# pdlfs/old-vpic

Measured on AMD Instinct MI355X. Metric: particle-pushes/sec (full step: advance_p + sort when due + field solve + glue), higher is better.
Workload: dtype f32

## Files before the change

### old-vpic_amd/csrc/push.hip

```cpp
#include "push_device.h"
#include "record_offsets.h"
#include <cstdlib>
#include <cstring>
#include <cstddef>
#include <vector>
#include <algorithm>

namespace vpichip {

struct PushParams {
  float qdt_2mc, cdt_dx, cdt_dy, cdt_dz;
  int np;
  int iters;
  int sy, sz;
  int idx_base;
  unsigned *crossed;
  const int *tpart, *ttail; int ntx, nty, ntiles, n_sorted; unsigned mul_sy, sh_sy, mul_sz, sh_sz;
  const int *tile_list; int n_launch, tail_chunks;
  int nx, ny, nz;
  int follow;
  double acc_scale;
  int *hist; int ntz;
  ParticlesK out; int *next;
  int stage;
// ... 63 lines not shown
struct MissList { int key[MISS_CAP]; float v[MISS_CAP][12]; int total; };

__device__ __forceinline__ void flush_misses(MissList *ml, int &n_miss, float *g_acc, int lane) {
  if (n_miss > 0) {
    __builtin_amdgcn_fence(__ATOMIC_ACQ_REL, "workgroup");
    const int entry = lane / 12, k = lane - entry * 12;
    if (entry < n_miss) atomicAdd(g_acc + (size_t)ml->key[entry] * 12 + k, ml->v[entry][k]);
    if (lane == 0) ml->total += n_miss;
    __builtin_amdgcn_fence(__ATOMIC_ACQ_REL, "workgroup");
    n_miss = 0;
  }
}

struct HistK { int *hist; unsigned *s_cnt; TileK tk; };
template <class W>
__device__ __forceinline__ void hist_count(const HistK &h, int key, int wbase, int sy, int sz, const TileDiv &td) {
  const int slot = slot_of<W>(key, wbase, sy, sz, td);
  if (slot >= 0) atomicAdd(&h.s_cnt[slot >> 1], 1u << ((slot & 1) << 4));
  else atomicAdd(&h.hist[sort_key<true>(key, h.tk)], 1);
}

template <class W>
__device__ __forceinline__ void deposit_run(const bool tail, float (&a)[12], int key, int lane, typename W::acc_t *s_acc, float *g_acc,
                                            int wbase, int sy, int sz, const TileDiv &td, MissList *ml, int &n_miss, const int pre_slot = -2) {
  const int slot = pre_slot != -2 ? pre_slot : slot_of<W>(key, wbase, sy, sz, td);
  if constexpr (is_det<W>::value) {
    if (tail) deposit12<true, W>(s_acc, g_acc, key, slot, a, td.scale);
    return;
  }
  if (tail && slot >= 0) deposit12<true, W>(s_acc, g_acc, key, slot, a);
  const bool miss = tail && slot < 0;
  const unsigned long long mm = __ballot(miss);
  if (mm) {
    if (miss) moments_to_terms(a, a);
    const int cnt = __popcll(mm);
    if (cnt > MISS_CAP) {
      if (miss) deposit12<true, W>(s_acc, g_acc, key, -1, a);
      if (lane == 0) ml->total += cnt;
      } else {
      if (n_miss + cnt > MISS_CAP) flush_misses(ml, n_miss, g_acc, lane);
      if (miss) {
        const int e = n_miss + mbcnt64(mm);
        ml->key[e] = key;
#pragma unroll
        for (int k = 0; k < 12; k++) ml->v[e][k] = a[k];
      }
      n_miss += cnt;
    }
  }
}

template <int BLOCK, class W>
__device__ __forceinline__ void run_deposit(float (&a)[12], int key, int lane, typename W::acc_t *s_acc, float *g_acc,
                                            int wbase, int sy, int sz, const TileDiv &td, MissList *ml, int &n_miss,
                                            const HistK *hk = nullptr, const bool counted = false, const int given_slot = -2) {
  static_assert(BLOCK == 1 || BLOCK == 2 || BLOCK == 4 || BLOCK == 8 || BLOCK == 16 || BLOCK == 64, "scan width");
  if (BLOCK == 1) {
    deposit_run<W>(key >= 0, a, key, lane, s_acc, g_acc, wbase, sy, sz, td, ml, n_miss);
    return;
  }
  const int prev = __builtin_amdgcn_update_dpp(-2, key, 0x138 , 0xf, 0xf, false);
  const unsigned long long block_heads = BLOCK == 64 ? 0ull : BLOCK == 16 ? 0x0001000100010001ull : BLOCK == 8 ? 0x0101010101010101ull
                                       : BLOCK == 4 ? 0x1111111111111111ull : 0x5555555555555555ull;
  const unsigned long long heads = __ballot(prev != key) | block_heads;
  const unsigned long long below = heads & ((2ull << lane) - 1ull);
  const int d = lane - (63 - __clzll((long long)below));
  const float f1 = d >= 1 ? 1.f : 0.f;
  SEG_STEP12(a, f1, "row_shr:1 row_mask:0xf bank_mask:0xf bound_ctrl:1");
  if (BLOCK >= 4) {
    const float f2 = d >= 2 ? 1.f : 0.f;
    SEG_STEP12(a, f2, "row_shr:2 row_mask:0xf bank_mask:0xf bound_ctrl:1");
  }
  if (BLOCK >= 8) {
    const float f4 = d >= 4 ? 1.f : 0.f;
    SEG_STEP12(a, f4, "row_shr:4 row_mask:0xf bank_mask:0xf bound_ctrl:1");
  }
  if (BLOCK >= 16) {
    const float f8 = d >= 8 ? 1.f : 0.f;
    SEG_STEP12(a, f8, "row_shr:8 row_mask:0xf bank_mask:0xf bound_ctrl:1");
  }
  if (BLOCK == 64) {
    const int r = lane & 15;
    const float f16 = d > r ? 1.f : 0.f;
    const float f32 = d > (lane & 31) ? 1.f : 0.f;
    SEG_STEP12(a, f16, "row_bcast:15 row_mask:0xa bank_mask:0xf");
    SEG_STEP12(a, f32, "row_bcast:31 row_mask:0xc bank_mask:0xf");
  }
  asm volatile("s_nop 1");
  const bool tail = (lane == 63) || ((heads >> ((lane + 1) & 63)) & 1ull);
  if (hk) {
    const int slot = slot_of<W>(key, wbase, sy, sz, td);
    const unsigned long long inc = __ballot(counted);
    const unsigned long long run = ((2ull << lane) - 1ull) & ~((1ull << (lane - d)) - 1ull);
    const int n = __popcll(inc & run);
    if (tail && key >= 0 && n) {
      if (slot >= 0) atomicAdd(&hk->s_cnt[slot >> 1], (unsigned)n << ((slot & 1) << 4));
      else atomicAdd(&hk->hist[sort_key<true>(key, hk->tk)], n);
    }
    deposit_run<W>(tail && key >= 0, a, key, lane, s_acc, g_acc, wbase, sy, sz, td, ml, n_miss, slot);
    return;
  }
  deposit_run<W>(tail && key >= 0, a, key, lane, s_acc, g_acc, wbase, sy, sz, td, ml, n_miss, given_slot);
}

template <int BLOCK, class W>
__device__ __forceinline__ void run_deposit_fixed(const float (&a)[12], int key, int lane, typename W::acc_t *s_acc, float *g_acc,
                                                  int wbase, int sy, int sz, const TileDiv &td, MissList *ml, int &n_miss) {
  static_assert(BLOCK == 16, "runs of at most 16 lanes, within a DPP row");
  unsigned long long v[12];
#pragma unroll
  for (int k = 0; k < 12; k++) v[k] = to_fixed(a[k], td.scale);
  const int prev = __builtin_amdgcn_update_dpp(-2, key, 0x138 , 0xf, 0xf, false);
  const unsigned long long heads = __ballot(prev != key) | 0x0001000100010001ull;
  const unsigned long long below = heads & ((2ull << lane) - 1ull);
  const int d = lane - (63 - __clzll((long long)below));
#pragma unroll
  for (int step = 1; step < 16; step <<= 1) {
    const bool on = d >= step;
#pragma unroll
    for (int k = 0; k < 12; k++) {
      const int lo = (int)(unsigned)v[k], hi = (int)(unsigned)(v[k] >> 32);
      const int tl = step == 1 ? __builtin_amdgcn_update_dpp(0, lo, 0x111 , 0xf, 0xf, true)
                   : step == 2 ? __builtin_amdgcn_update_dpp(0, lo, 0x112, 0xf, 0xf, true)
                   : step == 4 ? __builtin_amdgcn_update_dpp(0, lo, 0x114, 0xf, 0xf, true)
                               : __builtin_amdgcn_update_dpp(0, lo, 0x118, 0xf, 0xf, true);
      const int th = step == 1 ? __builtin_amdgcn_update_dpp(0, hi, 0x111, 0xf, 0xf, true)
                   : step == 2 ? __builtin_amdgcn_update_dpp(0, hi, 0x112, 0xf, 0xf, true)
                   : step == 4 ? __builtin_amdgcn_update_dpp(0, hi, 0x114, 0xf, 0xf, true)
                               : __builtin_amdgcn_update_dpp(0, hi, 0x118, 0xf, 0xf, true);
      const unsigned long long t = ((unsigned long long)(unsigned)th << 32) | (unsigned long long)(unsigned)tl;
      v[k] += on ? t : 0ull;
    }
  }
  const bool tail = key >= 0 && ((lane == 63) || ((heads >> ((lane + 1) & 63)) & 1ull));
  if (tail) {
    const int slot = slot_of<W>(key, wbase, sy, sz, td);
    unsigned long long *g64 = reinterpret_cast<unsigned long long *>(g_acc) + (size_t)key * 12;
#pragma unroll
    for (int k = 0; k < 12; k++) {
      if (slot >= 0) atomicAdd(&s_acc[k * W::NSLOT_PAD + slot], v[k]); else atomicAdd(&g64[k], v[k]);
    }
  }
  asm volatile("" ::: "memory");
}

constexpr int WAVES = PUSH_THREADS / 64;

#ifndef VPIC_HIP_MQW
#define VPIC_HIP_MQW 64
#endif
static_assert(VPIC_HIP_MQW >= 64, "a pass can yield 64 cell-crossers: the queue must hold them once it has been drained");
constexpr int MQW = VPIC_HIP_MQW;
struct WaveQueue { float4 pos_i[MQW]; float4 disp_idx[MQW]; float q[MQW]; };
constexpr int FLIP_SHIFT = 28;

__device__ __forceinline__ float fast_rsq(float x) { return __builtin_amdgcn_rsqf(x); }
__device__ __forceinline__ float fast_rcp(float x) { return __builtin_amdgcn_rcpf(x); }

template <class W>
__device__ __forceinline__ void mover_streak12(float *a, float q, float mx, float my, float mz, float sx, float sy, float sz) {
  if constexpr (is_det<W>::value) {
    const float v5 = (float)((double)(q * sx * sy * sz) * (1. / 3.));
    streak12(a, q, mx, my, mz, sx, sy, sz, v5);
  } else {
    streak12_moments(a, q, mx, my, mz, sx, sy, sz);
  }
}

constexpr int STAGE_CAP = 2;
template <bool CHARGELESS> struct StageRounds { static constexpr int value = CHARGELESS ? 2 : 1; };
struct StagePark { int base[STAGE_CAP], qb[STAGE_CAP]; unsigned cm_lo[STAGE_CAP], cm_hi[STAGE_CAP], act_lo[STAGE_CAP], act_hi[STAGE_CAP]; };
constexpr int STAGED_BIT = 31;
struct Straggler { float4 pos_i, disp_idx; float q; bool live; unsigned long long again; };

template <bool FAST, class W, bool HIST = false, bool STAGE = false, bool WIDE = false>
__device__ __forceinline__ int drain_wave(const ParticlesK &p, const int rel, WaveQueue *mq, const int n_mq,
                                          const int lane, typename W::acc_t *s_acc, float *g_acc, const int wbase,
                                          const DrainParams *dp, const int ablate, const int max_round, const int idx_base,
                                          MissList *ml, int &n_miss, const double det_scale = 0, const HistK *hk = nullptr, Straggler *sg = nullptr) {
  if (ablate & 64) return 0;
  typedef int int8v __attribute__((ext_vector_type(8)));
  typedef int int4v __attribute__((ext_vector_type(4)));
  int8v d0, d1; int4v d2;
  asm volatile("s_load_dwordx8 %0, %3, 0x0\n\ts_load_dwordx8 %1, %3, 0x20\n\ts_load_dwordx4 %2, %3, 0x40\n\ts_waitcnt lgkmcnt(0)"
               : "=&s"(d0), "=&s"(d1), "=&s"(d2) : "s"(dp));
  static_assert(offsetof(DrainParams, pbc) == 0x20 && offsetof(DrainParams, pm) == 0x40 && sizeof(DrainParams) == 0x50, "DrainParams layout");
  const int gnx = d0[0], gny = d0[1], gnz = d0[2], gsy = d0[3], gsz = d0[4], grank = d0[5], max_nm = d0[6];
  const unsigned mul_sz = (unsigned)d0[7], mul_sy = (unsigned)d1[6], sh_sz = (unsigned)d1[7] >> 8, sh_sy = (unsigned)d1[7] & 255u;
  const int pb0 = d1[0], pb1 = d1[1], pb2 = d1[2], pb3 = d1[3], pb4 = d1[4], pb5 = d1[5];
  const TileDiv td = {mul_sy, sh_sy, mul_sz, sh_sz, det_scale};
  typedef __attribute__((address_space(1))) vpic_particle_mover_t *global_mover_ptr;
  typedef __attribute__((address_space(1))) int *global_int_ptr;
  const global_mover_ptr pm = (global_mover_ptr)(((unsigned long long)(unsigned)d2[1] << 32) | (unsigned)d2[0]);
  const global_int_ptr nm_counter = (global_int_ptr)(((unsigned long long)(unsigned)d2[3] << 32) | (unsigned)d2[2]);
  int n_again = 0;
  for (int base = 0; base < n_mq; base += 64) {
    const int k = base + lane;
    bool live = k < n_mq;
    const int kq = live ? k : 0;
    const float4 c0 = mq->pos_i[kq], c2 = mq->disp_idx[kq];
    const float q = mq->q[kq];
    vpic_particle_mover_t m; m.dispx = c2.x; m.dispy = c2.y; m.dispz = c2.z; m.i = __float_as_int(c2.w);
    const int idx = m.i;
    const unsigned o4 = word_offset(idx, rel);
    float dx = c0.x, dy = c0.y, dz = c0.z;
    int flips = (__float_as_int(c0.w) >> FLIP_SHIFT) & 7;
    const bool staged = STAGE && live && (__float_as_int(c0.w) >> STAGED_BIT) & 1;
    int pi = live ? (__float_as_int(c0.w) & ((1 << FLIP_SHIFT) - 1)) : -1, cx = 0, cy = 0, cz = 0;
    if (live) {
      cz = (int)(__umulhi((unsigned)pi, mul_sz) >> sh_sz); const int rem = pi - cz * gsz;
      cy = (int)(__umulhi((unsigned)rem, mul_sy) >> sh_sy); cx = rem - cy * gsy;
    }
    const bool mine = live;
    bool stuck = false;
    const bool w0 = pb0 != grank, w1 = pb1 != grank, w2 = pb2 != grank, w3 = pb3 != grank, w4 = pb4 != grank, w5 = pb5 != grank;
    const bool r0 = pb0 == VPIC_REFLECT_PARTICLES, r1 = pb1 == VPIC_REFLECT_PARTICLES, r2 = pb2 == VPIC_REFLECT_PARTICLES,
               r3 = pb3 == VPIC_REFLECT_PARTICLES, r4 = pb4 == VPIC_REFLECT_PARTICLES, r5 = pb5 == VPIC_REFLECT_PARTICLES;
    for (int round = 0; round < max_round && __ballot(live); round++) {
      const bool up0 = m.dispx > 0, up1 = m.dispy > 0, up2 = m.dispz > 0;
      const float s_dir0 = up0 ? 1.f : -1.f, s_dir1 = up1 ? 1.f : -1.f, s_dir2 = up2 ? 1.f : -1.f;
      const float big = (float)3.4e38;
      float t0, t1, t2;
      if (FAST) {
        t0 = (fabsf(m.dispx) < 7.9e-31f) ? big : (s_dir0 - dx) * fast_rcp(m.dispx);
        t1 = (fabsf(m.dispy) < 7.9e-31f) ? big : (s_dir1 - dy) * fast_rcp(m.dispy);
        t2 = (fabsf(m.dispz) < 7.9e-31f) ? big : (s_dir2 - dz) * fast_rcp(m.dispz);
      } else {
        t0 = (m.dispx == 0) ? big : div_normal(s_dir0 - dx, m.dispx);
        t1 = (m.dispy == 0) ? big : div_normal(s_dir1 - dy, m.dispy);
        t2 = (m.dispz == 0) ? big : div_normal(s_dir2 - dz, m.dispz);
      }
      float v3 = 2.f;
      const bool lt0 = t0 < v3; v3 = lt0 ? t0 : v3;
      const bool lt1 = t1 < v3; v3 = lt1 ? t1 : v3;
      const bool lt2 = t2 < v3; v3 = lt2 ? t2 : v3;
      const bool ty2 = lt2, ty1 = lt1 && !lt2, ty0 = lt0 && !lt1 && !lt2;
      const bool moved_on = lt0 || lt1 || lt2;
      v3 *= 0.5f;
      const float s_dispx = m.dispx * v3, s_dispy = m.dispy * v3, s_dispz = m.dispz * v3;
      const float s_midx = dx + s_dispx, s_midy = dy + s_dispy, s_midz = dz + s_dispz;
      float a[12];
      mover_streak12<W>(a, q, s_midx, s_midy, s_midz, s_dispx, s_dispy, s_dispz);
      const int key = live ? pi : -1;
      const bool e0 = up0 ? (cx == gnx) : (cx == 1), e1 = up1 ? (cy == gny) : (cy == 1), e2 = up2 ? (cz == gnz) : (cz == 1);
      const bool hi = ty0 ? up0 : ty1 ? up1 : up2;
      const bool edge = ty0 ? e0 : ty1 ? e1 : e2;
      const bool wcode = hi ? (ty0 ? w3 : ty1 ? w4 : w5) : (ty0 ? w0 : ty1 ? w1 : w2);
      const bool rcode = hi ? (ty0 ? r3 : ty1 ? r4 : r5) : (ty0 ? r0 : ty1 ? r1 : r2);
      const bool wall = live && moved_on && edge && wcode;
      const bool refl = wall && rcode, stop = wall && !rcode;
      const bool hop = live && moved_on && !wall;
      if (live) {
        m.dispx -= s_dispx; m.dispy -= s_dispy; m.dispz -= s_dispz;
        dx += s_dispx + s_dispx; dy += s_dispy + s_dispy; dz += s_dispz + s_dispz;
        const float dir = ty0 ? s_dir0 : ty1 ? s_dir1 : s_dir2;
        const float face = hop ? -dir : dir;
        dx = ty0 ? face : dx; dy = ty1 ? face : dy; dz = ty2 ? face : dz;
        const int sgn = hi ? 1 : -1;
        const int nm1 = ty0 ? gnx - 1 : ty1 ? gny - 1 : gnz - 1;
        const int stride = ty0 ? 1 : ty1 ? gsy : gsz;
        const int dc = hop ? (edge ? -sgn * nm1 : sgn) : 0;
        pi += dc * stride;
        cx += ty0 ? dc : 0; cy += ty1 ? dc : 0; cz += ty2 ? dc : 0;
      }
      if (__ballot(refl)) {
        if (refl && ty0) { flips ^= 1; m.dispx = -m.dispx; }
        if (refl && ty1) { flips ^= 2; m.dispy = -m.dispy; }
        if (refl && ty2) { flips ^= 4; m.dispz = -m.dispz; }
      }
      stuck = stuck || stop;
      live = hop || refl;
      if (ablate & 32) {}
      else run_deposit<W::DRAIN_BLOCK, W>(a, key, lane, s_acc, g_acc, wbase, gsy, gsz, td, ml, n_miss);
      {
        const float n0 = ((m.dispx > 0) ? 1.f : -1.f) - dx, n1 = ((m.dispy > 0) ? 1.f : -1.f) - dy, n2 = ((m.dispz > 0) ? 1.f : -1.f) - dz;
        const float d0 = m.dispx + m.dispx, d1 = m.dispy + m.dispy, d2 = m.dispz + m.dispz;
        const bool h0 = (m.dispx > 0) ? (n0 < d0) : (m.dispx < 0) ? (n0 > d0) : false;
        const bool h1 = (m.dispy > 0) ? (n1 < d1) : (m.dispy < 0) ? (n1 > d1) : false;
        const bool h2 = (m.dispz > 0) ? (n2 < d2) : (m.dispz < 0) ? (n2 > d2) : false;
        const bool fin = live && !(h0 || h1 || h2);
        if (__ballot(fin)) {
          float b[12];
          mover_streak12<W>(b, q, dx + m.dispx, dy + m.dispy, dz + m.dispz, m.dispx, m.dispy, m.dispz);
          const int fkey = fin ? pi : -1;
          if (fin) {
            dx += m.dispx + m.dispx; dy += m.dispy + m.dispy; dz += m.dispz + m.dispz;
            live = false;
          }
          if (ablate & 32) {}
          else run_deposit<W::DRAIN_BLOCK, W>(b, fkey, lane, s_acc, g_acc, wbase, gsy, gsz, td, ml, n_miss);
        }
      }
    }
    const unsigned long long again = __ballot(live);
    if (STAGE) {
      sg->live = live; sg->again = again; sg->q = q;
      sg->pos_i = make_float4(dx, dy, dz, __int_as_float(pi | (flips << FLIP_SHIFT)));
      sg->disp_idx = make_float4(m.dispx, m.dispy, m.dispz, __int_as_float(idx));
      if (staged) mq->pos_i[k] = make_float4(dx, dy, dz, __int_as_float(live ? -1 : pi));
    } else
    if (live) {
      const int d = mbcnt64(again);
      mq->pos_i[d] = make_float4(dx, dy, dz, __int_as_float(pi | (flips << FLIP_SHIFT)));
      mq->disp_idx[d] = make_float4(m.dispx, m.dispy, m.dispz, __int_as_float(idx));
      mq->q[d] = q;
    }
    n_again = __popcll(again);
    if (mine && !live) {
#ifdef VPIC_HIP_ABLATION
      if (ablate & 256) {} else
#endif
      if (!staged) {
        if (WIDE) { rec4 v; v.x = dx; v.y = dy; v.z = dz; v.w = __int_as_float(pi); __builtin_nontemporal_store(v, rec_at(p.r, (unsigned)idx)); }
        else str_nt(p.r, o4 << 2, dx, dy, dz, pi);
      }
      if (HIST) hist_count<W>(*hk, pi, wbase, gsy, gsz, td);
      if (flips) {
        asm volatile("s_waitcnt vmcnt(0)" ::: "memory");
        if (flips & 1) stf(p.ux, o4, -ldf(p.ux, o4));
        if (flips & 2) stf(p.uy, o4, -ldf(p.uy, o4));
        if (flips & 4) stf(p.uz, o4, -ldf(p.uz, o4));
      }
      if (stuck) {
        const int gs = __hip_atomic_fetch_add(nm_counter, 1, __ATOMIC_RELAXED, __HIP_MEMORY_SCOPE_AGENT);
        if (gs < max_nm) { pm[gs].dispx = m.dispx; pm[gs].dispy = m.dispy; pm[gs].dispz = m.dispz; pm[gs].i = m.i + idx_base; }
      }
    }
  }
  return n_again;
}

constexpr int TAIL_CHUNK = 1024;

template <bool CHARGELESS = false, bool FAST = false, int WIN = 0, bool HIST = false, bool SORT = false>
#ifndef VPIC_HIP_PUSH_VGPRS
#define VPIC_HIP_PUSH_VGPRS 80
#endif
__global__ __launch_bounds__(PUSH_THREADS) __attribute__((amdgpu_num_vgpr(VPIC_HIP_PUSH_VGPRS)))
void advance_p_kernel(ParticlesK p, const float4 *__restrict__ fi, float *__restrict__ g_acc,
                      const DrainParams *__restrict__ dp, const PushParams P) {
  typedef Window<WIN> W;
  typedef typename W::acc_t acc_t;
  constexpr bool TILE = W::TILE;
  constexpr bool DET = is_det<W>::value;
  constexpr bool UNORDERED = WIN == 3 || WIN == 5 || WIN == 6;
  constexpr int WX = W::WX, NSLOT_PAD = W::NSLOT_PAD;
  __shared__ acc_t s_acc[12 * NSLOT_PAD];
  __shared__ WaveQueue s_mq[WAVES];
  __shared__ MissList s_miss[WAVES];
  __shared__ int s_wbase;
  __shared__ unsigned s_cnt[HIST ? (NSLOT_PAD + 1) / 2 : SORT ? NSLOT_PAD : 1];
  constexpr bool STAGE = (WIN == 3 || CHARGELESS) && !HIST && !SORT;
  __shared__ StagePark s_park[STAGE ? WAVES : 1];
  static_assert(!HIST || WIN == 2, "the histogram of the next sort is taken in tile order, by cell");
  static_assert(!SORT || (WIN == 2 && !HIST && !CHARGELESS), "the sort inside the push: tile order by cell, its counts taken by the push before");

#ifdef VPIC_HIP_ABLATION
  const int ablate = P.ablate | (CHARGELESS ? (1 | 8 | 16 | 32) : 0);
#else
  constexpr int ablate = CHARGELESS ? (1 | 8 | 16 | 32) : 0;
#endif
  const int tid = threadIdx.x;
  const int lane = tid & 63;
  const int wave = __builtin_amdgcn_readfirstlane(tid >> 6);
  const unsigned chunk = xcd_block(blockIdx.x, gridDim.x);
  int first, last, wave_span = 0, tile_base = NO_WINDOW;
  int first2 = 0, last2 = 0;
  int bx0 = 0, by0 = 0, bz0 = 0;
  if (TILE) {
    if (chunk < (unsigned)P.n_launch) {
      const unsigned tile = P.tile_list ? (unsigned)P.tile_list[chunk] : chunk;
      first = min(P.tpart[tile * TILE_CELLS], P.np);
      last = min(P.tpart[tile * TILE_CELLS + TILE_CELLS], P.np);
      if (P.ttail) {
        first2 = min(P.n_sorted + P.ttail[tile * TILE_CELLS], P.np);
        last2 = min(P.n_sorted + P.ttail[tile * TILE_CELLS + TILE_CELLS], P.np);
      }
      const unsigned txy = tile % (unsigned)(P.ntx * P.nty), tz = tile / (unsigned)(P.ntx * P.nty);
      const unsigned tx = txy % (unsigned)P.ntx, ty = txy / (unsigned)P.ntx;
      tile_base = TILE_EDGE * ((int)tx + P.sy * (int)ty + P.sz * (int)tz);
      bx0 = TILE_EDGE * (int)tx; by0 = TILE_EDGE * (int)ty; bz0 = TILE_EDGE * (int)tz;
    } else {
      if (chunk - (unsigned)P.n_launch >= (unsigned)P.tail_chunks) return;
      first = min(P.n_sorted, P.np) + (int)(chunk - (unsigned)P.n_launch) * TAIL_CHUNK;
      last = min(first + TAIL_CHUNK, P.np);
    }
    if (first >= last && first2 >= last2) return;
  } else {
    wave_span = 64 * P.iters;
    if ((long long)chunk * (WAVES * wave_span) >= P.np) return;
    first = (int)chunk * (WAVES * wave_span);
    last = P.np;
  }

#ifndef VPIC_HIP_FOLLOW
#define VPIC_HIP_FOLLOW 1
#endif
  constexpr int FOLLOW_REACH = 3;
  int sample = -1;
  bool follow = false;
  if (TILE && VPIC_HIP_FOLLOW && tile_base != NO_WINDOW) {
    unsigned flag = 0;
    if (P.follow < 0) asm volatile("s_load_dword %0, %1, 0x8\n\ts_waitcnt lgkmcnt(0)" : "=s"(flag) : "s"(P.crossed));
    follow = P.follow > 0 || flag == 1u;
  }
  if (follow && wave == 0 && last > first)
    sample = record_cell(p.r, (long long)first + (int)(((long long)lane * (last - first)) >> 6));
  if (!CHARGELESS)
    for (int k = tid; k < 12 * NSLOT_PAD; k += PUSH_THREADS) s_acc[k] = 0;
  if (HIST)
    for (int k = tid; k < (NSLOT_PAD + 1) / 2; k += PUSH_THREADS) s_cnt[k] = 0;
  if (SORT)
    for (int k = tid; k < NSLOT_PAD; k += PUSH_THREADS) s_cnt[k] = 0;
  if (TILE) {
    if (follow) {
      if (wave == 0) {
        const bool have = sample >= 0;
        const int cz = (int)(__umulhi((unsigned)max(sample, 0), P.mul_sz) >> P.sh_sz), rem = max(sample, 0) - cz * P.sz;
        const int cy = (int)(__umulhi((unsigned)rem, P.mul_sy) >> P.sh_sy), cx = rem - cy * P.sy;
        int best[3];
#pragma unroll
        for (int a = 0; a < 3; a++) {
          const int c = a == 0 ? cx : a == 1 ? cy : cz, b0 = a == 0 ? bx0 : a == 1 ? by0 : bz0, n = a == 0 ? P.nx : a == 1 ? P.ny : P.nz;
          const int hi = max(n - 4, 0);
          int pick = min(max(b0, 0), hi), top = -1;
#pragma unroll
          for (int t = 0; t < 2 * FOLLOW_REACH + 1; t++) {
            const int d = (t & 1) ? -((t + 1) >> 1) : (t >> 1);
            const int b = min(max(b0 + d, 0), hi);
            const int cover = __popcll(__ballot(have && c >= b && c <= b + 5)), inner = __popcll(__ballot(have && c > b && c < b + 5));
            const int score = 2 * cover + inner;
            if (score > top) { top = score; pick = b; }
          }
          best[a] = pick;
        }
        if (lane == 0) s_wbase = best[0] + P.sy * best[1] + P.sz * best[2];
      }
    } else if (tid == 0) s_wbase = tile_base;
  } else if (DET) {
    if (tid == 0) s_wbase = NO_WINDOW;
  } else if (!CHARGELESS && wave == 0) {
    const int chunk_n = min(WAVES * wave_span, P.np - first);
    const int sidx = first + (int)(((long long)lane * chunk_n) >> 6);
    const int k0 = record_cell(p.r, sidx);
    int rank = 0;
    for (int l = 0; l < 64; l++) {
      const int kl = __builtin_amdgcn_readlane(k0, l);
      rank += (kl < k0 || (kl == k0 && l < lane)) ? 1 : 0;
    }
    const unsigned long long is_med = __ballot(rank == 31);
    const int m = __builtin_amdgcn_readlane(k0, __ffsll((long long)is_med) - 1) - WX / 2 + WMARGIN;
    if (lane == 0) s_wbase = m - WMARGIN;
  }
  __syncthreads();
  const int wbase = s_wbase;
  const int gsy = P.sy, gsz = P.sz;
  WaveQueue *mq = &s_mq[wave];
  MissList *ml = &s_miss[wave];
  if (lane == 0) ml->total = 0;
  int n_miss = 0;
  int n_mq = 0, n_crossed = 0;

  TileDiv td = {0u, 0u, 0u, 0u, 0.0};
  if (TILE) { td.mul_sy = P.mul_sy; td.sh_sy = P.sh_sy; td.mul_sz = P.mul_sz; td.sh_sz = P.sh_sz; }
  if (DET) td.scale = P.acc_scale;
  TileDiv vtd = td;
  int vsy = gsy, vsz = gsz;
  if (TILE && !DET) {
    vtd.mul_sy = (unsigned)in_vgpr((int)P.mul_sy); vtd.sh_sy = (unsigned)in_vgpr((int)P.sh_sy);
    vtd.mul_sz = (unsigned)in_vgpr((int)P.mul_sz); vtd.sh_sz = (unsigned)in_vgpr((int)P.sh_sz);
    vsy = in_vgpr(gsy); vsz = in_vgpr(gsz);
  }
  HistK hk;
  if (HIST || SORT) {
    hk.hist = P.hist; hk.s_cnt = s_cnt;
    hk.tk.sy = P.sy; hk.tk.sz = P.sz; hk.tk.ntx = P.ntx; hk.tk.nty = P.nty; hk.tk.ntz = P.ntz; hk.tk.ntiles = P.ntiles;
    hk.tk.mul_sy = P.mul_sy; hk.tk.sh_sy = P.sh_sy; hk.tk.mul_sz = P.mul_sz; hk.tk.sh_sz = P.sh_sz;
    hk.tk.mx = P.nx - 1; hk.tk.my = P.ny - 1; hk.tk.mz = P.nz - 1;
  }

  float st0x = 0.f, st0y = 0.f, st0z = 0.f, st1x = 0.f, st1y = 0.f, st1z = 0.f;
  int st0i = 0, st1i = 0;
  int n_pend = 0;
  const bool stage = STAGE && P.stage != 0;
  StagePark *park = &s_park[STAGE ? wave : 0];
  ParticlesK pw = p;
  int rel = 0;
  auto drain_release = [&](const bool all) -> int {
    Straggler sg; sg.live = false; sg.again = 0ull;
    int n_back = 0;
    if (n_mq > 0) {
      __builtin_amdgcn_fence(__ATOMIC_RELEASE, "workgroup");
      n_back = drain_wave<FAST, W, HIST, STAGE>(pw, rel, mq, n_mq, lane, s_acc, g_acc, wbase, dp, ablate, all ? (1 << 30) : StageRounds<CHARGELESS>::value, P.idx_base, ml, n_miss, td.scale, &hk, &sg);
      __builtin_amdgcn_fence(__ATOMIC_ACQ_REL, "workgroup");
    }
#pragma unroll
    for (int j = 0; j < STAGE_CAP; j++) {
      if (j >= n_pend) break;
      const int pb = __builtin_amdgcn_readfirstlane(park->base[j]), qb = __builtin_amdgcn_readfirstlane(park->qb[j]);
      const unsigned long long cmj = ((unsigned long long)(unsigned)__builtin_amdgcn_readfirstlane((int)park->cm_hi[j]) << 32) | (unsigned)__builtin_amdgcn_readfirstlane((int)park->cm_lo[j]);
      const unsigned long long actj = ((unsigned long long)(unsigned)__builtin_amdgcn_readfirstlane((int)park->act_hi[j]) << 32) | (unsigned)__builtin_amdgcn_readfirstlane((int)park->act_lo[j]);
      float fx = j ? st1x : st0x, fy = j ? st1y : st0y, fz = j ? st1z : st0z;
      int fi_ = j ? st1i : st0i;
// ... 137 lines not shown
    bool crosser;
    float sux, suy, suz;
    float spx = 0.f, spy = 0.f, spz = 0.f;
    {
      const unsigned o4 = word_offset(idx, sfirst);
      float v0, v1, v2, v3, v4, v5;
      if (FAST) {
        const float hax = qdt_2mc * __builtin_fmaf(dz, __builtin_fmaf(dy, fe_x.w, fe_x.z), __builtin_fmaf(dy, fe_x.y, fe_x.x));
        const float hay = qdt_2mc * __builtin_fmaf(dx, __builtin_fmaf(dz, fe_y.w, fe_y.z), __builtin_fmaf(dz, fe_y.y, fe_y.x));
        const float haz = qdt_2mc * __builtin_fmaf(dy, __builtin_fmaf(dx, fe_z.w, fe_z.z), __builtin_fmaf(dx, fe_z.y, fe_z.x));
        const float cbx = __builtin_fmaf(dx, fb0.y, fb0.x), cby = __builtin_fmaf(dy, fb0.w, fb0.z), cbz = __builtin_fmaf(dz, fb1.y, fb1.x);
        ux += hax; uy += hay; uz += haz;
        v0 = qdt_2mc * fast_rsq(__builtin_fmaf(ux, ux, __builtin_fmaf(uy, uy, __builtin_fmaf(uz, uz, one))));
        v1 = __builtin_fmaf(cbx, cbx, __builtin_fmaf(cby, cby, cbz * cbz));
        v2 = (v0 * v0) * v1;
        v3 = v0 * __builtin_fmaf(v2, __builtin_fmaf(v2, two_fifteenths, one_third), one);
        v4 = (v3 + v3) * fast_rcp(__builtin_fmaf(v1, v3 * v3, one));
        v0 = __builtin_fmaf(v3, __builtin_fmaf(uy, cbz, -(uz * cby)), ux);
        v1 = __builtin_fmaf(v3, __builtin_fmaf(uz, cbx, -(ux * cbz)), uy);
        v2 = __builtin_fmaf(v3, __builtin_fmaf(ux, cby, -(uy * cbx)), uz);
        ux = __builtin_fmaf(v4, __builtin_fmaf(v1, cbz, -(v2 * cby)), ux);
        uy = __builtin_fmaf(v4, __builtin_fmaf(v2, cbx, -(v0 * cbz)), uy);
        uz = __builtin_fmaf(v4, __builtin_fmaf(v0, cby, -(v1 * cbx)), uz);
        ux += hax; uy += hay; uz += haz;
      } else {
        const float hax = qdt_2mc * ((fe_x.x + dy * fe_x.y) + dz * (fe_x.z + dy * fe_x.w));
        const float hay = qdt_2mc * ((fe_y.x + dz * fe_y.y) + dx * (fe_y.z + dz * fe_y.w));
        const float haz = qdt_2mc * ((fe_z.x + dx * fe_z.y) + dy * (fe_z.z + dx * fe_z.w));
        const float cbx = fb0.x + dx * fb0.y;
        const float cby = fb0.z + dy * fb0.w;
        const float cbz = fb1.x + dz * fb1.y;
        ux += hax; uy += hay; uz += haz;
        v0 = div_normal(qdt_2mc, sqrt_normal(one + (ux * ux + (uy * uy + uz * uz))));
        v1 = cbx * cbx + (cby * cby + cbz * cbz);
        v2 = (v0 * v0) * v1;
        v3 = v0 * (one + v2 * (one_third + v2 * two_fifteenths));
        v4 = div_normal(v3, one + v1 * (v3 * v3));
        v4 += v4;
        v0 = ux + v3 * (uy * cbz - uz * cby);
        v1 = uy + v3 * (uz * cbx - ux * cbz);
        v2 = uz + v3 * (ux * cby - uy * cbx);
        ux += v4 * (v1 * cbz - v2 * cby);
        uy += v4 * (v2 * cbx - v0 * cbz);
        uz += v4 * (v0 * cby - v1 * cbx);
        ux += hax; uy += hay; uz += haz;
      }
      sux = ux; suy = uy; suz = uz;
      if (FAST) v0 = fast_rsq(__builtin_fmaf(ux, ux, __builtin_fmaf(uy, uy, __builtin_fmaf(uz, uz, one))));
      else v0 = div_normal(one, sqrt_normal(one + (ux * ux + (uy * uy + uz * uz))));
      ux *= cdt_dx; uy *= cdt_dy; uz *= cdt_dz;
      ux *= v0; uy *= v0; uz *= v0;
      v0 = dx + ux; v1 = dy + uy; v2 = dz + uz;
      v3 = v0 + ux; v4 = v1 + uy; v5 = v2 + uz;
      const bool incell = (ablate & 2) || fmaxf(fmaxf(fabsf(v3), fabsf(v4)), fabsf(v5)) <= one;
      crosser = active && !incell;
      if (SORT) {
        dst = __shfl(sort_b, sort_head) + (lane - sort_head);
        if (active) {
          const unsigned d4 = (unsigned)dst << 2;
          stf(P.out.ux, d4, sux); stf(P.out.uy, d4, suy); stf(P.out.uz, d4, suz);
          rec4 v; v.x = incell ? v3 : dx; v.y = incell ? v4 : dy; v.z = incell ? v5 : dz; v.w = __int_as_float(key);
          *rec_at(P.out.r, (unsigned)dst) = v;
          stf(P.out.q, d4, q);
        }
      } else
      if (STAGE && stage) {
        if (!TILE || active) { stf(pw.ux, o4, sux); stf(pw.uy, o4, suy); stf(pw.uz, o4, suz); }
        spx = incell ? v3 : dx; spy = incell ? v4 : dy; spz = incell ? v5 : dz;
      } else
      if ((!TILE || active) && !(ablate & 128)) {
        stf_nt(pw.ux, o4, sux); stf_nt(pw.uy, o4, suy); stf_nt(pw.uz, o4, suz);
        str(pw.r, o4 << 2, incell ? v3 : dx, incell ? v4 : dy, incell ? v5 : dz, key);
      }
      if (!CHARGELESS && !(ablate & 1)) {
        const float qd = (incell && active) ? q : 0.f;
        if constexpr (is_det<W>::value) streak12(a, qd, v0, v1, v2, ux, uy, uz, qd * ux * uy * uz * one_third);
        else streak12_moments(a, qd, v0, v1, v2, ux, uy, uz);
      } else {
#pragma unroll
        for (int k = 0; k < 12; k++) a[k] = 0.f;
      }
    }
    if constexpr (WIN == 4) run_deposit_fixed<16, W>(a, key, lane, s_acc, g_acc, wbase, gsy, gsz, td, ml, n_miss);
    else
    if (!CHARGELESS) run_deposit<UNORDERED ? 1 : TILE ? TILE_MAIN_BLOCK : MAIN_BLOCK, W>(a, (UNORDERED && crosser) ? -1 : key, lane, s_acc, g_acc, wbase, vsy, vsz, vtd, ml, n_miss,
                                                                                            HIST ? &hk : nullptr, active && !crosser, SORT ? sort_slot : -2);
    {
      const unsigned long long cm = __ballot(crosser);
      const int cnt = __popcll(cm);
      n_crossed += cnt;
      if constexpr (STAGE) {
        int phase = (n_mq + cnt > MQW) ? 0 : 1, attempt = 0;
#pragma unroll 1
        for (;;) {
          if (phase == 1) {
            if (crosser) {
              const int d = n_mq + mbcnt64(cm);
              mq->pos_i[d] = make_float4(dx, dy, dz, __int_as_float(stage ? (key | (1 << STAGED_BIT)) : key));
              mq->disp_idx[d] = make_float4(ux, uy, uz, __int_as_float(idx));
              mq->q[d] = q;
            }
            if (stage) {
              if (n_pend == 0) { st0x = spx; st0y = spy; st0z = spz; st0i = key; } else { st1x = spx; st1y = spy; st1z = spz; st1i = key; }
              const unsigned long long act = __ballot(!TILE || active);
              if (lane == 0) {
                park->base[n_pend] = base; park->qb[n_pend] = n_mq;
                park->cm_lo[n_pend] = (unsigned)cm; park->cm_hi[n_pend] = (unsigned)(cm >> 32);
                park->act_lo[n_pend] = (unsigned)act; park->act_hi[n_pend] = (unsigned)(act >> 32);
              }
              n_pend++;
            }
            n_mq += cnt;
            if (n_mq < 64 && n_pend < STAGE_CAP) break;
          }
          n_mq = drain_release(phase == 0 && attempt > 0);
          if (phase == 1) break;
          attempt++;
          if (n_mq + cnt <= MQW) phase = 1;
        }
      } else {
      int attempt = 0;
#pragma unroll 1
      for (int phase = (n_mq + cnt > MQW) ? 0 : 1; phase < 2;) {
        if (phase == 1) {
          if (crosser) {
            const int d = n_mq + mbcnt64(cm);
            mq->pos_i[d] = make_float4(dx, dy, dz, __int_as_float(key));
            mq->disp_idx[d] = make_float4(ux, uy, uz, __int_as_float(SORT ? dst : idx));
            mq->q[d] = q;
          }
          n_mq += cnt;
          if (n_mq < 64) break;
        }
        const int n_now = min(n_mq, 64);
        __builtin_amdgcn_fence(__ATOMIC_RELEASE, "workgroup");
        const int cap = (phase == 0 && attempt > 0) ? (1 << 30) : 1;
        const int n_back = drain_wave<FAST, W, HIST, false, SORT>(SORT ? P.out : pw, rel, mq, n_now, lane, s_acc, g_acc, wbase, dp, ablate, cap, P.idx_base, ml, n_miss, td.scale, &hk);
            const int n_left = n_mq - n_now;
        const int src = lane < n_left ? 64 + lane : 0;
        const float4 t0 = mq->pos_i[src], t2 = mq->disp_idx[src];
        const float t1 = mq->q[src];
        __builtin_amdgcn_fence(__ATOMIC_ACQ_REL, "workgroup");
        if (lane < n_left) { const int d = n_back + lane; mq->pos_i[d] = t0; mq->disp_idx[d] = t2; mq->q[d] = t1; }
        n_mq = n_back + n_left;
        if (phase == 0) { attempt++; if (n_mq + cnt <= MQW) phase = 1; }
        else phase = 2;
      }
      }
    }
  }
  }
  __builtin_amdgcn_fence(__ATOMIC_RELEASE, "workgroup");
  if constexpr (STAGE) n_mq = drain_release(true);
  else
  drain_wave<FAST, W, HIST, false, SORT>(SORT ? P.out : pw, rel, mq, n_mq, lane, s_acc, g_acc, wbase, dp, ablate, 1 << 30, P.idx_base, ml, n_miss, td.scale, &hk);
  if (!CHARGELESS && !DET) flush_misses(ml, n_miss, g_acc, lane);

  if (lane == 0 && n_crossed) atomicAdd(P.crossed + (blockIdx.x & 255u) * 16u, (unsigned)n_crossed);
  if (!CHARGELESS && lane == 0 && ml->total) atomicAdd(P.crossed + (blockIdx.x & 255u) * 16u + 1u, (unsigned)ml->total);

  __syncthreads();
  if (ablate & 8) return;
  if (HIST && wbase != NO_WINDOW) {
    for (int slot = tid; slot < W::NSLOT; slot += PUSH_THREADS) {
      const unsigned n = (s_cnt[slot >> 1] >> ((slot & 1) << 4)) & 0xffffu;
      const int lx = slot % WX, lyz = slot / WX, ly = lyz % WX, lz = lyz / WX;
      if (n) atomicAdd(&P.hist[sort_key<true>(wbase + lx + gsy * ly + gsz * lz, hk.tk)], (int)n);
    }
  }
  const int k = tid % 12, c0 = tid / 12;
  if constexpr (DET) {
    if (TILE && wbase != NO_WINDOW && tid < 12 * FLUSH_CELLS) {
      unsigned long long *g64 = reinterpret_cast<unsigned long long *>(g_acc);
      for (int cell = c0; cell < W::NSLOT; cell += FLUSH_CELLS) {
        const unsigned long long v = (unsigned long long)s_acc[k * NSLOT_PAD + cell];
        const int lx = cell % WX, lyz = cell / WX, ly = lyz % WX, lz = lyz / WX;
        if (v) atomicAdd(g64 + (size_t)(wbase + lx + gsy * ly + gsz * lz) * 12 + k, v);
      }
    }
  } else if constexpr (TILE) {
    if (wbase != NO_WINDOW && tid < 12 * FLUSH_CELLS) {
      const TermSigns sg = term_signs(k & 3);
      const acc_t *src = s_acc + (k & ~3) * NSLOT_PAD;
      for (int cell = c0; cell < W::NSLOT; cell += FLUSH_CELLS) {
        const float v = (float)term_of(sg, src[cell], src[NSLOT_PAD + cell], src[2 * NSLOT_PAD + cell], src[3 * NSLOT_PAD + cell]);
        const int lx = cell % WX, lyz = cell / WX, ly = lyz % WX, lz = lyz / WX;
        if (v != 0.f) atomicAdd(g_acc + (size_t)(wbase + lx + gsy * ly + gsz * lz) * 12 + k, v);
      }
    }
  } else if (tid < 12 * FLUSH_CELLS) {
    const TermSigns sg = term_signs(k & 3);
#pragma unroll
    for (int s = 0; s < NSEG; s++) {
      const int seg_base = wbase + ((s == 0) ? 0 : (s == 1) ? gsy : (s == 2) ? -gsy : (s == 3) ? gsz : -gsz);
      const acc_t *src = s_acc + (k & ~3) * NSLOT_PAD + s * WX;
      float *dst = g_acc + (size_t)seg_base * 12 + k;
      for (int cell = c0; cell < WX; cell += FLUSH_CELLS) {
        const float v = (float)term_of(sg, src[cell], src[NSLOT_PAD + cell], src[2 * NSLOT_PAD + cell], src[3 * NSLOT_PAD + cell]);
        if (v != 0.f) atomicAdd(dst + cell * 12, v);
      }
    }
  }
}

__global__ __launch_bounds__(256) void publish_counter_kernel(unsigned *__restrict__ host_word, unsigned *__restrict__ dev_shards, unsigned cycle, unsigned long long follow_from) {
  __shared__ unsigned s_sum[4];
  unsigned v = dev_shards[threadIdx.x * 16];
  dev_shards[threadIdx.x * 16] = 0;
  for (int off = 32; off; off >>= 1) v += __shfl_down(v, off);
  if ((threadIdx.x & 63) == 0) s_sum[threadIdx.x >> 6] = v;
  __syncthreads();
  if (threadIdx.x == 0) host_word[0] = s_sum[0] + s_sum[1] + s_sum[2] + s_sum[3];
  __syncthreads();
  v = dev_shards[threadIdx.x * 16 + 1];
  dev_shards[threadIdx.x * 16 + 1] = 0;
  for (int off = 32; off; off >>= 1) v += __shfl_down(v, off);
  if ((threadIdx.x & 63) == 0) s_sum[threadIdx.x >> 6] = v;
  __syncthreads();
  if (threadIdx.x == 0) {
    const unsigned missed = s_sum[0] + s_sum[1] + s_sum[2] + s_sum[3];
    host_word[3] = missed; host_word[4] = cycle;
    const unsigned state = dev_shards[2];
    if (state == 0u && (unsigned long long)missed > follow_from) dev_shards[2] = 1u;
    else if (state == 1u && (unsigned long long)missed > 4ull * follow_from) dev_shards[2] = 2u;
  }
}

__global__ __launch_bounds__(256) void fuse_check_kernel(const int *__restrict__ cursor, const int *__restrict__ starts, int n1, unsigned *__restrict__ bad) {
  const int k = blockIdx.x * 256 + threadIdx.x;
  const bool wrong = k + 1 < n1 && cursor[k] != starts[k + 1];
  const unsigned long long m = __ballot(wrong);
  if (m && (threadIdx.x & 63) == 0) atomicAdd(bad, (unsigned)__popcll(m));
}

__global__ void fuse_clear_kernel(unsigned *__restrict__ w) { *w = 0; }
__global__ void fuse_publish_kernel(unsigned *__restrict__ host_word, const unsigned *__restrict__ dev_word) { *host_word = *dev_word; }

int k_sort_check(Engine *e, Species &s, const int *starts, int n1) {
  unsigned *word = reinterpret_cast<unsigned *>(e->counters + 201);
  hipLaunchKernelGGL(fuse_clear_kernel, dim3(1), dim3(1), 0, e->stream, word);
  hipLaunchKernelGGL(fuse_check_kernel, dim3((n1 + 255) / 256), dim3(256), 0, e->stream, (const int *)e->sort_next, starts, n1, word);
  hipLaunchKernelGGL(fuse_publish_kernel, dim3(1), dim3(1), 0, e->stream, s.crossed_host_dev + PW_SORT_CHECK, (const unsigned *)word);
  VH_CHECK(hipGetLastError());
  return 0;
}

static int begin_profile(Engine *e, int64_t particles, int kind = 0, int species = -1) {
  if (!e->profile) return -1;
  if (e->ev_used == e->ev_pool.size()) {
    hipEvent_t a, b;
    if (hipEventCreate(&a) != hipSuccess || hipEventCreate(&b) != hipSuccess) return -1;
    e->ev_pool.push_back({a, b});
    e->ev_particles.push_back(0); e->ev_kind.push_back(0); e->ev_species.push_back(-1);
  }
  const int k = (int)e->ev_used++;
  e->ev_particles[k] = particles; e->ev_kind[k] = (char)kind; e->ev_species[k] = species;
  (void)hipEventRecord(e->ev_pool[k].first, e->stream);
  return k;
}

extern "C" int vpic_hip_push_plan(int64_t np, int iters, int64_t *start, int32_t *count, uint32_t *grid, int max_segments) {
  if (np < 0 || iters < 1 || iters > PUSH_ITERS || max_segments < 1) return -1;
  const int64_t per_chunk = (int64_t)PUSH_THREADS * iters;
  int64_t seg = push_segment_particles(per_chunk);
  if (np <= ((int64_t)1 << 30) && (np % 64 == 0 || np <= ((int64_t)1 << 30) - 64)) seg = (np + per_chunk - 1) / per_chunk * per_chunk;
  int n = 0;
  for (int64_t at = 0; at < np; at += seg, n++) {
    if (n >= max_segments) return -1;
    const int64_t c = np - at < seg ? np - at : seg;
    start[n] = at; count[n] = (int32_t)c;
    const uint32_t chunks = (uint32_t)((c + per_chunk - 1) / per_chunk);
    grid[n] = (chunks + 7u) & ~7u;
  }
  return n;
}

static int ensure_tile_lists(Engine *e) {
  if (e->tile_list[0] || e->tile_list_n[0] < 0) return 0;
  const TileK tk = make_tile_k(e->gk);
  bool shared[6]; bool any = false;
  for (int f = 0; f < 6; f++) { shared[f] = e->gk.pbc[f] >= 0 && e->gk.pbc[f] != e->gk.rank; any = any || shared[f]; }
  if (!any) { e->tile_list_n[0] = -1; return 0; }
  std::vector<int> list[2];
  for (int tz = 0; tz < tk.ntz; tz++) for (int ty = 0; ty < tk.nty; ty++) for (int tx = 0; tx < tk.ntx; tx++) {
    const bool edge = (shared[0] && tx == 0) || (shared[3] && tx == tk.ntx - 1) || (shared[1] && ty == 0) || (shared[4] && ty == tk.nty - 1) ||
                      (shared[2] && tz == 0) || (shared[5] && tz == tk.ntz - 1);
    list[edge ? 0 : 1].push_back((tz * tk.nty + ty) * tk.ntx + tx);
  }
  for (int k = 0; k < 2; k++) {
    VH_CHECK(hipMalloc(&e->tile_list[k], sizeof(int) * std::max<size_t>(list[k].size(), 1)));
    if (!list[k].empty()) VH_CHECK(hipMemcpy(e->tile_list[k], list[k].data(), sizeof(int) * list[k].size(), hipMemcpyHostToDevice));
    e->tile_list_n[k] = (int)list[k].size();
  }
  return 0;
}

template <bool CHARGELESS, int WIN = 0, bool HIST = false, bool SORT = false>
static void launch_push(bool fast, unsigned grid, hipStream_t stream, const ParticlesK &p, const float4 *fi, float *g_acc, DrainParams *d, const PushParams &P) {
  if (fast) hipLaunchKernelGGL((advance_p_kernel<CHARGELESS, true, WIN, HIST, SORT>), dim3(grid), dim3(PUSH_THREADS), 0, stream, p, fi, g_acc, d, P);
  else hipLaunchKernelGGL((advance_p_kernel<CHARGELESS, false, WIN, HIST, SORT>), dim3(grid), dim3(PUSH_THREADS), 0, stream, p, fi, g_acc, d, P);
}

int k_advance_p(Engine *e, Species &s, bool async, int phase) {
  const vpic_hip_grid_t &g = e->grid;
  PushParams P;
  P.qdt_2mc = (float)(0.5 * s.q_m * g.dt / g.cvac);
  P.cdt_dx = g.cvac * g.dt * g.rdx;
  P.cdt_dy = g.cvac * g.dt * g.rdy;
  P.cdt_dz = g.cvac * g.dt * g.rdz;
  P.np = (int)s.np;
  P.sy = e->gk.sy; P.sz = e->gk.sz;
#ifdef VPIC_HIP_ABLATION
  P.ablate = e->knobs.ablate;
#endif
// ... 293 lines not shown
```

Baseline: 61.81 billion.

## Rebalance end-of-push cell-crosser queues across wavefronts before final drain

```diff
diff --git a/old-vpic_amd/csrc/push.hip b/old-vpic_amd/csrc/push.hip
--- a/old-vpic_amd/csrc/push.hip
+++ b/old-vpic_amd/csrc/push.hip
@@ -239,6 +239,10 @@
 static_assert(VPIC_HIP_MQW >= 64, "a pass can yield 64 cell-crossers: the queue must hold them once it has been drained");
 constexpr int MQW = VPIC_HIP_MQW;
 struct WaveQueue { float4 pos_i[MQW]; float4 disp_idx[MQW]; float q[MQW]; };
+#ifndef VPIC_HIP_ENDGAME_ROUNDS
+#define VPIC_HIP_ENDGAME_ROUNDS 1
+#endif
+constexpr int ENDGAME_ROUNDS = VPIC_HIP_ENDGAME_ROUNDS;
 constexpr int FLIP_SHIFT = 28;
 
 __device__ __forceinline__ float fast_rsq(float x) { return __builtin_amdgcn_rsqf(x); }
@@ -436,6 +440,7 @@
   __shared__ WaveQueue s_mq[WAVES];
   __shared__ MissList s_miss[WAVES];
   __shared__ int s_wbase;
+  __shared__ int s_nq[WAVES];
   __shared__ unsigned s_cnt[HIST ? (NSLOT_PAD + 1) / 2 : SORT ? NSLOT_PAD : 1];
   constexpr bool STAGE = (WIN == 3 || CHARGELESS) && !HIST && !SORT;
   __shared__ StagePark s_park[STAGE ? WAVES : 1];
@@ -879,14 +884,44 @@
   }
   __builtin_amdgcn_fence(__ATOMIC_RELEASE, "workgroup");
   if constexpr (STAGE) n_mq = drain_release(true);
-  else
-  drain_wave<FAST, W, HIST, false, SORT>(SORT ? P.out : pw, rel, mq, n_mq, lane, s_acc, g_acc, wbase, dp, ablate, 1 << 30, P.idx_base, ml, n_miss, td.scale, &hk);
+  else {
+    static_assert(WAVES * 64 == PUSH_THREADS && (WAVES & (WAVES - 1)) == 0, "a batch per wavefront, turns by masking");
+    const unsigned wg = blockIdx.x;
+    int turn = (int)((wg + (wg >> 2) + (wg >> 4) + (wg >> 6) + (wg >> 8) + (wg >> 10) + (wg >> 12) + (wg >> 14) + (wg >> 16)) & (WAVES - 1));
+#pragma unroll 1
+    for (;; turn++) {
+      if (lane == 0) s_nq[wave] = n_mq;
+      __syncthreads();
+      const int batch = (wave - turn) & (WAVES - 1);
+      const int g = batch * 64 + lane;
+      int T = 0, from = 0, lo = 0;
+#pragma unroll
+      for (int w = 0; w < WAVES; w++) {
+        const int n = __builtin_amdgcn_readfirstlane(s_nq[w]);
+        if (g >= T + n) { from = w + 1; lo = T + n; }
+        T += n;
+      }
+      if (T == 0) break;
+      const bool pool = MQW == 64 || T <= 64 * WAVES;
+      const bool take = pool && g < T;
+      const WaveQueue *const src = &s_mq[take ? from : 0];
+      const int at = take ? g - lo : 0;
+      const float4 t0 = src->pos_i[at], t2 = src->disp_idx[at];
+      const float t1 = src->q[at];
+      __syncthreads();
+      if (take) { mq->pos_i[lane] = t0; mq->disp_idx[lane] = t2; mq->q[lane] = t1; }
+      if (pool) n_mq = min(max(T - batch * 64, 0), 64);
+      __builtin_amdgcn_fence(__ATOMIC_RELEASE, "workgroup");
+      if (n_mq > 0)
+        n_mq = drain_wave<FAST, W, HIST, false, SORT>(SORT ? P.out : pw, rel, mq, n_mq, lane, s_acc, g_acc, wbase, dp, ablate, pool ? ENDGAME_ROUNDS : (1 << 30), P.idx_base, ml, n_miss, td.scale, &hk);
+    }
+  }
   if (!CHARGELESS && !DET) flush_misses(ml, n_miss, g_acc, lane);
 
   if (lane == 0 && n_crossed) atomicAdd(P.crossed + (blockIdx.x & 255u) * 16u, (unsigned)n_crossed);
   if (!CHARGELESS && lane == 0 && ml->total) atomicAdd(P.crossed + (blockIdx.x & 255u) * 16u + 1u, (unsigned)ml->total);
 
-  __syncthreads();
+  if constexpr (STAGE) __syncthreads();
   if (ablate & 8) return;
   if (HIST && wbase != NO_WINDOW) {
     for (int slot = tid; slot < W::NSLOT; slot += PUSH_THREADS) {
```

Measured after the change: 58.47 billion. 0.946x the previous value.
